# KrishTanna28/Real-Time-Video-Deepfake-Detection

Hardware: AMD Instinct MI355X
Metric: face-crops/sec (224x224 crops through EfficientNet-B0 classify) (higher is better)
Workload: dtype f32; 1 GPU; configs[1]: batch=256 random 224x224 crops, EfficientNet-B0 fp32 inference; batch_per_gpu=256, parallelism=frame-shard x1, no data-path collective, forwards_in_flight=2

## Files before the change

### real-time-video-deepfake-detection_amd/csrc/b0_kernels.h

```cpp
#pragma once
#include <hip/hip_runtime.h>

#include <string>

namespace dfd {

typedef __bf16 bf16_t;

enum Act { ACT_NONE = 0, ACT_SWISH = 1, ACT_RELU = 2, ACT_PRELU = 3 };

template <typename XT>
void launch_stem(const float* x_nchw, const float* w , const float* b,
                 XT* y, int n, hipStream_t s);

template <typename XT>
void launch_stem_dw(const float* x_nchw, const unsigned short* ws3, int plane, int Kp, const float* bs, const float* Wd,
                    const float* bd, XT* Y, float* P, XT* stem_out, int n, int* tiles, hipStream_t s);

void launch_pointwise(const float* X, const float* W, const float* bias, const float* gate,
                      const float* R, float* Y, int M, int K, int N, int HW, int act,
                      hipStream_t s);

struct ConvGeom {
    int H = 0, W = 0, Ho = 0, Wo = 0, Cin = 0, ksize = 1, stride = 1, pad = 0, dil = 1;
};

bool launch_conv_gemm(const float* X, const float* W, const float* bias, const float* R, float* Y,
                      int n_img, const ConvGeom& g, int Cout, int act, bool res_first, hipStream_t s);

size_t split_weights_count(int N, int K);
void launch_split_weights(const float* W, unsigned short* out, int N, int K, hipStream_t s, bool transposed = false);
bool split_gemm_supports(int K, int N);
bool split_gemm_thin_supports(int K, int N, int HW);
struct S6Table;
S6Table* s6_table_create();
void s6_table_destroy(S6Table* t);
void s6_table_set_force(S6Table* t, int idx);
void s6_table_set_tuning(S6Table* t, bool on);
int s6_table_measured(const S6Table* t);
int s6_max_candidates();
long long s6_chunk_rows(long long M, long long row_bytes, long long HW);
std::string s6_table_export(const S6Table* t);
int s6_table_import(S6Table* t, const char* text, size_t len);
template <typename XT>
bool launch_pointwise_split(S6Table* tab, const XT* X, const unsigned short* W3, const float* bias, const float* gate,
                            const XT* R, XT* Y, int M, int K, int N, int HW, int act, int planes, hipStream_t s);
template <typename XT>
bool launch_conv_gemm_split(S6Table* tab, const XT* X, const unsigned short* W3, const float* bias, const XT* R,
                            XT* Y, int n_img, const ConvGeom& g, int Cout, int act, bool res_first, int planes, hipStream_t s);

template <typename XT>
bool launch_depthwise(const XT* X, const float* W , const float* bias, XT* Y,
                      float* P, int n, int H, int C, int k, int stride, int pad_lo,
                      int* tiles, hipStream_t s);
int depthwise_tiles(int H, int C, int k, int stride);
template <typename XT>
bool launch_mbconv_front(const XT* Xin, int Cin, const unsigned short* We3, int plane, int Kp, const float* Wef, const float* be,
                         const float* Wd, const float* bd, XT* Y, float* P, int n, int H, int C, int k, int stride,
                         int pad_lo, int* tiles, hipStream_t s, bool late = false);
int mbconv_tiles(int H, int C, int k, int stride, int Cin, bool late = false);

void launch_se(const float* P, int tiles, float inv_hw, const float* w1, const float* b1,
               const float* w2t, const float* b2, float* gate, int n, int C, int c_se,
               hipStream_t s);

template <typename XT>
void launch_avgpool(const XT* X, float* Y, int n, int hw, int C, hipStream_t s);
void launch_bf16_to_f32(const bf16_t* x, float* y, size_t n, hipStream_t s);

}
```

### real-time-video-deepfake-detection_amd/csrc/b0_plan.hip

```cpp
#include <algorithm>

#include "b0_kernels.h"
#include "dfd_common.h"

namespace dfd {

thread_local std::string g_create_error;

int fail(dfd_handle* h, int code, const char* fmt, ...) {
    char buf[512];
    va_list ap;
    va_start(ap, fmt);
    vsnprintf(buf, sizeof buf, fmt, ap);
    va_end(ap);
    if (h) h->err = buf;
    else g_create_error = buf;
    return code;
}

namespace {

struct Stage { int rep, k, s, e, ci, co; };
const Stage kStages[] = {{1, 3, 1, 1, 32, 16}, {2, 3, 2, 6, 16, 24}, {2, 5, 2, 6, 24, 40},
                         {3, 3, 2, 6, 40, 80}, {3, 5, 1, 6, 80, 112}, {4, 5, 2, 6, 112, 192},
// ... 187 lines not shown
    }
    if ((rc = tap_out(h, tap, "stem", io0, (size_t)n * 112 * 112 * 32))) return rc;
    XT* cur = io0;
    XT* nxt = io1;
    int bi = 0;
    for (const B0Block& b : P.blocks) {
        const int m_in = n * b.h_in * b.h_in, m_out = n * b.h_out * b.h_out;
        const std::string q = "b" + std::to_string(bi);
        const XT* dw_in = cur;
        int tiles = 0;
        bool fused = false;
        const unsigned short* we3 = nullptr;
        const bool late_here = h->fuse_late && !((h->fuse_late_skip >> bi) & 1u);
        if (b.expand != 1 && h->fuse_expand && mbconv_tiles(b.h_in, b.c_exp, b.kernel, b.stride, b.c_in, late_here) > 0 &&
            !(we3 = split_weights(h, b.exp_w, b.c_exp, b.c_in))) return DFD_ERR_HIP;
        if (we3 && launch_mbconv_front<XT>(cur, b.c_in, we3, (int)split_weights_count(b.c_exp, b.c_in), (b.c_in + 63) / 64 * 64,
                                           b.exp_w, b.exp_b, b.dw_w, b.dw_b, dwbuf, h->pool, n, b.h_in, b.c_exp,
                                           b.kernel, b.stride, b.pad_lo, &tiles, s, late_here)) {
            fused = true;
            mk.mark(layer_name(bi, "dw"));
            if (tap && tap->name && q + ".exp" == tap->name)
                return fail(h, DFD_ERR_STATE, "tap '%s': the expanded tensor is not materialised when expand is fused "
                                              "(dfd_set_option(h, \"fuse_expand\", 0))", tap->name);
        }
        if (!fused && b.expand != 1) {
            if ((rc = pointwise_t<XT>(h, cur, b.exp_w, b.exp_b, nullptr, nullptr, expbuf, m_in, b.c_in, b.c_exp,
                                      b.h_in * b.h_in, ACT_SWISH))) return rc;
            mk.mark(layer_name(bi, "exp"));
            if ((rc = tap_out(h, tap, q + ".exp", expbuf, (size_t)m_in * b.c_exp))) return rc;
            dw_in = expbuf;
        }
        if (bi == 0 && stem_fused) {
            tiles = stem_tiles;
        } else if (!fused) {
            if (!launch_depthwise<XT>(dw_in, b.dw_w, b.dw_b, dwbuf, h->pool, n, b.h_in, b.c_exp, b.kernel,
                                      b.stride, b.pad_lo, &tiles, s))
                return fail(h, DFD_ERR_STATE, "no depthwise kernel for block %d", bi);
            mk.mark(layer_name(bi, "dw"));
        }
        if ((rc = tap_out(h, tap, q + ".dw", dwbuf, (size_t)m_out * b.c_exp))) return rc;
        launch_se(h->pool, tiles, 1.0f / (float)(b.h_out * b.h_out), b.se_w1, b.se_b1, b.se_w2, b.se_b2,
                  h->gate, n, b.c_exp, b.c_se, s);
        mk.mark(layer_name(bi, "se"));
        if ((rc = tap_out(h, tap, q + ".gate", h->gate, (size_t)n * b.c_exp))) return rc;
        if ((rc = pointwise_t<XT>(h, dwbuf, b.proj_w, b.proj_b, h->gate, b.skip ? cur : (const XT*)nullptr, nxt, m_out,
                                  b.c_exp, b.c_out, b.h_out * b.h_out, ACT_NONE))) return rc;
        mk.mark(layer_name(bi, "proj"));
        if ((rc = tap_out(h, tap, q + ".out", nxt, (size_t)m_out * b.c_out))) return rc;
        XT* t = cur; cur = nxt; nxt = t;
        ++bi;
    }
    const B0Block& last = P.blocks.back();
    const int hw = last.h_out * last.h_out;
    if ((rc = pointwise_t<XT>(h, cur, P.head_w, P.head_b, nullptr, nullptr, headbuf, n * hw, last.c_out, 1280, hw,
                              ACT_SWISH))) return rc;
    mk.mark("head");
    if ((rc = tap_out(h, tap, "head", headbuf, (size_t)n * hw * 1280))) return rc;
    launch_avgpool<XT>(headbuf, h->feat, n, hw, 1280, s);
    mk.mark("avgpool");
    if ((rc = tap_out(h, tap, "feat", h->feat, (size_t)n * 1280))) return rc;
    if (!logits_dev) return DFD_OK;
    if ((rc = pointwise(h, h->feat, P.fc1_w, P.fc1_b, nullptr, nullptr, h->fc1, n, 1280, 512, 1, ACT_RELU))) return rc;
    if ((rc = pointwise(h, h->fc1, P.fc2_w, P.fc2_b, nullptr, nullptr, h->fc2, n, 512, 256, 1, ACT_RELU))) return rc;
    launch_pointwise(h->fc2, P.fc3_w, P.fc3_b, nullptr, nullptr, logits_dev, n, 256, 1, 1, ACT_NONE, s);
    mk.mark("mlp");
    if ((rc = tap_out(h, tap, "logit", logits_dev, (size_t)n))) return rc;
    DFD_HIP_TRY(h, hipGetLastError());
    return DFD_OK;
}

float* b0_last_block_out(const dfd_handle* h) { return h->b0.blocks.size() % 2 == 0 ? h->io0 : h->io1; }

int b0_head_preact(dfd_handle* h, int n, void* z_out) {
    const B0Plan& P = h->b0;
    const B0Block& last = P.blocks.back();
    const int hw = last.h_out * last.h_out;
    if (h->act_bf16)
        return pointwise_t<bf16_t>(h, reinterpret_cast<const bf16_t*>(b0_last_block_out(h)), P.head_w, P.head_b, nullptr, nullptr,
                                   static_cast<bf16_t*>(z_out), n * hw, last.c_out, 1280, hw, ACT_NONE);
    return pointwise_t<float>(h, b0_last_block_out(h), P.head_w, P.head_b, nullptr, nullptr, static_cast<float*>(z_out),
                              n * hw, last.c_out, 1280, hw, ACT_NONE);
}

int b0_forward(dfd_handle* h, const float* x, int n, float* logits_dev, B0Tap* tap, B0Prof* prof) {
    if (n > 0) h->classifier_crops += (unsigned long long)n;
    return h->act_bf16 ? b0_forward_t<bf16_t>(h, x, n, logits_dev, tap, prof)
                       : b0_forward_t<float>(h, x, n, logits_dev, tap, prof);
}

}
```

### real-time-video-deepfake-detection_amd/csrc/dfd_api.hip

```cpp
#include "b0_kernels.h"
#include "dfd_common.h"

using namespace dfd;

namespace {

int dev_alloc(dfd_handle* h, size_t bytes, float** out) {
    void* p = nullptr;
    DFD_HIP_TRY(h, hipMalloc(&p, bytes ? bytes : 4));
    h->owned.push_back(p);
    *out = static_cast<float*>(p);
    return DFD_OK;
}

__global__ __launch_bounds__(256) void fill_pattern_kernel(float* __restrict__ x, size_t n) {
    const size_t i = (size_t)blockIdx.x * 256 + threadIdx.x;
    if (i >= n) return;
    uint32_t v = (uint32_t)i * 2654435761u;
    v ^= v >> 15; v *= 2246822519u; v ^= v >> 13;
    x[i] = ((float)(v >> 8) * (1.0f / 16777216.0f) - 0.5f) * 4.0f;
}

int create_impl(dfd_handle* h, int device, const void* blob, size_t blob_len, int max_batch) {
    int ndev = 0;
// ... 83 lines not shown
    }
    h->jpeg_stream = nullptr;
    if (h->aux_stream) {
        hipStreamSynchronize(h->aux_stream);
        hipStreamDestroy(h->aux_stream);
        hipEventDestroy(h->aux_go);
        hipEventDestroy(h->aux_done);
    }
    if (h->jpeg_host) hipHostFree(h->jpeg_host);
    if (h->mailbox) hipHostFree(h->mailbox);
    for (char* p : h->mailbox_old) hipHostFree(p);
    for (char* p : h->mailbox_old_prev) hipHostFree(p);
    if (h->ev0) hipEventDestroy(h->ev0);
    if (h->order_ev) hipEventDestroy(h->order_ev);
    if (h->ev1) hipEventDestroy(h->ev1);
    if (h->stream) hipStreamDestroy(h->stream);
    delete h;
}

}

extern "C" {

int dfd_abi_version(void) { return DFD_ABI_VERSION; }

int dfd_create(int device, const void* blob, size_t blob_len, int max_batch, dfd_handle** out) {
    if (!out) return fail(nullptr, DFD_ERR_ARG, "dfd_create: out is null");
    *out = nullptr;
    if (!blob || max_batch <= 0 || max_batch > 4096)
        return fail(nullptr, DFD_ERR_ARG, "dfd_create: blob is null or max_batch outside 1..4096");
    dfd_handle* h = new (std::nothrow) dfd_handle();
    if (!h) return fail(nullptr, DFD_ERR_ARG, "dfd_create: out of host memory");
    const int rc = create_impl(h, device, blob, blob_len, max_batch);
    if (rc != DFD_OK) {
        g_create_error = h->err;
        destroy_impl(h);
        return rc;
    }
    *out = h;
    return DFD_OK;
}

void dfd_destroy(dfd_handle* h) { destroy_impl(h); }

const char* dfd_last_error(const dfd_handle* h) { return h ? h->err.c_str() : g_create_error.c_str(); }

int dfd_max_batch(const dfd_handle* h) { return h ? h->max_batch : DFD_ERR_ARG; }

int dfd_set_option(dfd_handle* h, const char* name, int value) {
    if (!h || !name) return DFD_ERR_ARG;
    if (strcmp(name, "fuse_expand") == 0) { h->fuse_expand = value != 0; return DFD_OK; }
    if (strcmp(name, "fuse_late") == 0) { h->fuse_late = value != 0; return DFD_OK; }
    if (strcmp(name, "fuse_late_skip") == 0) { h->fuse_late_skip = (unsigned)value; return DFD_OK; }
    if (strcmp(name, "fuse_stem") == 0) { h->fuse_stem = value != 0; return DFD_OK; }
    if (strcmp(name, "split_gemm") == 0) { h->split_gemm = value != 0; return DFD_OK; }
    if (strcmp(name, "mtcnn") == 0) { h->use_mtcnn = value != 0; return DFD_OK; }
    if (strcmp(name, "overlap_forensics") == 0) { h->overlap_forensics = value != 0; return DFD_OK; }
    if (strcmp(name, "bf16_activations") == 0) { h->act_bf16 = value != 0; return DFD_OK; }
    if (strcmp(name, "bf16_weight_planes") == 0) {
        if (value != 1 && value != 3) return fail(h, DFD_ERR_ARG, "bf16_weight_planes must be 1 or 3");
        h->bf16_planes = value;
        return DFD_OK;
    }
    if (strcmp(name, "gemm_tile") == 0) { s6_table_set_force(h->gemm, value); return DFD_OK; }
    if (strcmp(name, "jpeg_device_entropy") == 0) { h->jpeg_device_entropy = value < 0 ? 0 : value; return DFD_OK; }
    if (strcmp(name, "jpeg_rounds") == 0) { h->jpeg_rounds = value; return DFD_OK; }
    if (strcmp(name, "jpeg_chunk_bytes") == 0) {
        if (value < 256 || value > (1 << 20) || (value & (value - 1))) return fail(h, DFD_ERR_ARG, "jpeg_chunk_bytes: a power of two in 256 .. 2^20");
        h->jpeg_chunk_bytes = value;
        return DFD_OK;
    }
    if (strcmp(name, "stream_priority") == 0) {
        if (value < -1 || value > 1) return fail(h, DFD_ERR_ARG, "stream_priority must be -1, 0 or 1");
        DFD_HIP_TRY(h, hipSetDevice(h->device));
        DFD_HIP_TRY(h, stream_sync(h));
        if (h->aux_stream) DFD_HIP_TRY(h, hipStreamSynchronize(h->aux_stream));
        if (h->copy_stream) DFD_HIP_TRY(h, hipStreamSynchronize(h->copy_stream));
        int least = 0, greatest = 0;
        DFD_HIP_TRY(h, hipDeviceGetStreamPriorityRange(&least, &greatest));
        const int prio = value > 0 ? greatest : (value < 0 ? least : (least + greatest) / 2);
        hipStream_t fresh = nullptr;
        DFD_HIP_TRY(h, hipStreamCreateWithPriority(&fresh, hipStreamNonBlocking, prio));
        hipStreamDestroy(h->stream);
        h->stream = fresh;
        return DFD_OK;
    }
    if (strcmp(name, "profile_stride") == 0) { h->prof_stride = value > 0 ? value : 1; return DFD_OK; }
    return fail(h, DFD_ERR_ARG, "unknown option '%s'", name);
}

int dfd_warmup(dfd_handle* h, int n_crops, int n_frames) {
    if (!h) return DFD_ERR_ARG;
    if (n_crops < 0 || n_crops > h->max_batch || n_frames < 0)
        return fail(h, DFD_ERR_ARG, "warmup: n_crops outside 0..%d or n_frames negative", h->max_batch);
    DFD_HIP_TRY(h, hipSetDevice(h->device));
    s6_table_set_tuning(h->gemm, true);
    int rc = DFD_OK;
    if (n_crops > 0) {
        const size_t cnt = (size_t)n_crops * 3 * 224 * 224;
        hipLaunchKernelGGL(fill_pattern_kernel, dim3((unsigned)((cnt + 255) / 256)), dim3(256), 0, h->stream, h->in_nchw, cnt);
        rc = b0_forward(h, h->in_nchw, n_crops, h->logits, nullptr, nullptr);
    }
    if (rc == DFD_OK && n_frames > 0) rc = ssd_warmup(h, n_frames);
    s6_table_set_tuning(h->gemm, false);
    if (rc) return rc;
    DFD_HIP_TRY(h, stream_sync(h));
// ... 192 lines not shown
```

### real-time-video-deepfake-detection_amd/csrc/dfd_common.h

```cpp
#pragma once
#include <hip/hip_runtime.h>

#include <cstdarg>
#include <cstdint>
#include <cstdio>
#include <cstring>
#include <map>
#include <string>
#include <vector>

#include "../../include/dfd_hip.h"
#include "blob_reader.h"
#include "imgproc_kernels.h"

namespace dfd {

struct ForensicState;
void forensic_destroy(dfd_handle* h);
struct FreqState;
void freq_destroy(dfd_handle* h);
struct SsdState;
int ssd_init(dfd_handle* h);
void ssd_destroy(dfd_handle* h);
int ssd_warmup(dfd_handle* h, int n_frames);
// ... 33 lines not shown
    float* out = nullptr;
    size_t capacity = 0, count = 0;
    bool found = false;
};
struct B0Prof {
    std::vector<hipEvent_t> events;
    std::vector<const char*> names;
    bool enabled = false;
};

}

struct dfd_handle {
    int device = 0;
    int max_batch = 0;
    hipStream_t stream = nullptr;
    hipEvent_t ev0 = nullptr, ev1 = nullptr;
    hipEvent_t order_ev = nullptr;
    char* mailbox = nullptr;
    size_t mailbox_cap = 0, mailbox_head = 0, mailbox_lap_end = 0;
    size_t mailbox_live = 0, mailbox_live_prev = 0;
    std::vector<char*> mailbox_old, mailbox_old_prev;
    hipStream_t aux_stream = nullptr;
    hipEvent_t aux_go = nullptr, aux_done = nullptr;
    bool overlap_forensics = true;
    hipStream_t copy_stream = nullptr;
    hipEvent_t copy_done[2] = {nullptr, nullptr}, slot_free[2] = {nullptr, nullptr};
    dfd::DevBuf stage[2];
    std::map<std::string, dfd::Tensor> tensors;
    std::vector<void*> owned;
    dfd::B0Plan b0;
    float *in_nchw = nullptr, *io0 = nullptr, *io1 = nullptr, *expbuf = nullptr, *dwbuf = nullptr;
    float *pool = nullptr, *gate = nullptr, *headbuf = nullptr, *feat = nullptr, *fc1 = nullptr,
          *fc2 = nullptr, *logits = nullptr;
    dfd::ColorTables color{};
    bool has_color = false;
    dfd::DevBuf frame_buf, lab_buf, crop_buf, lut_buf, desc_buf, u8_out, face_batch;
    dfd::DevBuf det_desc;
    int last_detections = 0;
    std::vector<char> crop_valid;
    int n_compact = 0;
    unsigned long long classifier_crops = 0;
    dfd::ForensicState* forensic = nullptr;
    dfd::FreqState* freq = nullptr;
    dfd::SsdState* ssd = nullptr;
    dfd::MtcnnState* mtcnn = nullptr;
    dfd::HaarState* haar = nullptr;
    dfd::CommState* comm = nullptr;
    bool use_mtcnn = true;
    bool fuse_stem = true;
    bool fuse_expand = true;
    bool fuse_late = true;
    unsigned fuse_late_skip = (1u << 8) | (1u << 9);
    bool split_gemm = true;
    bool act_bf16 = false;
    int bf16_planes = 3;
    dfd::DevBuf jpeg_work;
    dfd::DevBuf jpeg_raw[2];
    dfd::DevBuf jpeg_work2[2];
    hipStream_t jpeg_stream = nullptr;
    hipEvent_t jpeg_done[2] = {nullptr, nullptr}, frames_free[2] = {nullptr, nullptr};
    void* jpeg_host = nullptr;
    size_t jpeg_host_cap = 0;
    int jpeg_device_entropy = 2;
    int jpeg_rounds = 16;
    int jpeg_chunk_bytes = 512;
    unsigned long long jpeg_frames_device = 0, jpeg_frames_host = 0;
    dfd::DevBuf tap_buf;
    std::map<const float*, unsigned short*> wsplit;
    dfd::S6Table* gemm = nullptr;
    dfd::B0Prof prof;
    int prof_steps = 0;
    int prof_seen = 0, prof_stride = 1;
    std::string err;
};

namespace dfd {

extern thread_local std::string g_create_error;

int fail(dfd_handle* h, int code, const char* fmt, ...);

#define DFD_HIP_TRY(h, expr)                                                                    \
    do {                                                                                        \
        hipError_t _e = (expr);                                                                 \
        if (_e != hipSuccess)                                                                   \
            return dfd::fail((h), DFD_ERR_HIP, "%s failed: %s (%s:%d)", #expr, hipGetErrorString(_e), \
                             __FILE__, __LINE__);                                               \
    } while (0)

int ensure(dfd_handle* h, DevBuf* b, size_t bytes);
hipError_t stream_sync(dfd_handle* h);
int mailbox_h2d(dfd_handle* h, void* dst_dev, const void* src, size_t bytes);
const void* mailbox_d2h(dfd_handle* h, const void* src_dev, size_t bytes);
void copy_kernel_async(void* dst, const void* src, size_t bytes, hipStream_t s);
int color_tables_init(dfd_handle* h);

int forensics_run(dfd_handle* h, int stream_id, const uint8_t* frame_dev, int hh, int ww, int stride, int full,
                  double* scores_out, double* prob_out, double* stats_out);
int detect_run(dfd_handle* h, const uint8_t* frame_dev, int hh, int ww, int stride, float conf_thr, int32_t* xywh_out,
               float* conf_out, int max_out, int* n_out);
int haar_run(dfd_handle* h, const uint8_t* frame_dev, int hh, int ww, int stride, float scale_factor, int min_neighbors,
             int min_size, int32_t* xywh_out, int max_out, int* n_out, int* n_candidates, int* n_total = nullptr);
int preprocess_run(dfd_handle* h, const uint8_t* frame_dev, int hh, int ww, int stride, const int32_t* xywh, int n,
                   int apply_clahe, const size_t* frame_offs = nullptr, bool compact = false);
int classify_boxes(dfd_handle* h, const uint8_t* frame_dev, int hh, int ww, int stride, const int32_t* xywh, int m,
// ... 38 lines not shown
```

### real-time-video-deepfake-detection_amd/csrc/gemm_split.hip

```cpp
#include "gemm_split_impl.h"

#include <algorithm>
#include <cmath>
#include <cstdio>
#include <cstdlib>
#include <map>
#include <new>
#include <string>
#include <tuple>
#include <vector>

namespace dfd {

DFD_S6_INSTANTIATE(float, 3)

__global__ __launch_bounds__(256) void split_weights_kernel(const float* __restrict__ W, __bf16* __restrict__ out,
                                                            int N, int K, int Np, int Kp, int transposed) {
    const size_t i = (size_t)blockIdx.x * 256 + threadIdx.x, plane = (size_t)Np * Kp;
    if (i >= plane) return;
    const int n = (int)(i / Kp), k = (int)(i - (size_t)n * Kp);
    const float a = n < N && k < K ? (transposed ? W[(size_t)k * N + n] : W[(size_t)n * K + k]) : 0.f;
    const __bf16 h0 = (__bf16)a;
    const float r1 = a - (float)h0;
    const __bf16 h1 = (__bf16)r1;
// ... 35 lines not shown
            const double blocks = (double)t.mblocks * t.nblocks;
            const double useful = (double)tiles / ((double)t.nblocks * nt);
            const double rounds = std::max(1.0, std::ceil(blocks / 512.0));
            const double cost = rounds * (mt * nt + 1.5) / useful;
            if (cost < best_cost - 1e-9) { best_cost = cost; best = t; }
        }
    return best;
}

static std::vector<S6Tile> s6_candidates(int M, int K, int N, bool thin = false, bool wide = false) {
    const int tiles = (N + 15) / 16;
    std::vector<S6Tile> raw, out;
    for (int ks = 1; ks <= (K > 32 ? 2 : 1); ++ks)
        for (int mt = 1; mt <= 2; ++mt)
            for (int nt = 1; nt <= 8 && nt <= tiles; ++nt) raw.push_back(make_tile6(M, N, mt, nt, ks));
    for (int ks = 1; ks <= (K > 32 ? 2 : 1); ++ks)
        for (int nt = 2; nt <= 8 && nt <= tiles; ++nt) raw.push_back(make_tile(M, N, 0, 8, 1, 1, nt, ks));
#define DFD_S7_CAND(WMV, WNV, MTV, NTV) raw.push_back(make_tile(M, N, 1, WMV, WNV, MTV, NTV));
    DFD_S7_CONFIGS(DFD_S7_CAND)
#undef DFD_S7_CAND
    for (const S6Tile& t : raw) {
        const int bn_tiles = t.kind == 0 ? t.nt : t.wn * t.nt;
        if ((double)tiles / ((double)t.nblocks * bn_tiles) < 0.7) continue;
        if ((long long)t.mblocks * t.nblocks > (1 << 20)) continue;
        out.push_back(t);
    }
    if (out.empty()) out.push_back(make_tile6(M, N, 1, 1));
    if (wide)
    {
        for (int nt : {6, 4}) out.push_back(make_tile(M, N, 3, 4, 1, 2, nt, 1));
        out.push_back(make_tile(M, N, 3, 4, 1, 2, 4, 2));
    }
    if (thin)
        for (int bpc : {2, 3, 4, 6, 8, 12, 16, 24}) out.push_back(make_tile(M, N, 2, s8_waves(K), 1, 1, tiles, bpc));
    return out;
}

struct S6Key {
    int M, K, N, mode;
    bool operator<(const S6Key& o) const {
        return std::tie(M, K, N, mode) < std::tie(o.M, o.K, o.N, o.mode);
    }
};
struct S6Table {
    std::map<S6Key, S6Tile> tiles;
    int force = -1;
    bool tuning = false;
};

S6Table* s6_table_create() { return new (std::nothrow) S6Table(); }
void s6_table_destroy(S6Table* t) { delete t; }
void s6_table_set_force(S6Table* t, int idx) { if (t) t->force = idx; }
void s6_table_set_tuning(S6Table* t, bool on) { if (t) t->tuning = on; }
int s6_table_measured(const S6Table* t) {
    int n = 0;
    if (t) for (const auto& kv : t->tiles) n += kv.second.measured ? 1 : 0;
    return n;
}
std::string s6_table_export(const S6Table* t) {
    std::string out;
    if (!t) return out;
    char line[128];
    for (const auto& kv : t->tiles) {
        if (!kv.second.measured) continue;
        snprintf(line, sizeof line, "%d %d %d %d %d %d %d %d %d %d\n", kv.first.M, kv.first.K, kv.first.N, kv.first.mode,
                 kv.second.kind, kv.second.wm, kv.second.wn, kv.second.mt, kv.second.nt, kv.second.ks);
        out += line;
    }
    return out;
}
int s6_table_import(S6Table* t, const char* text, size_t len) {
    if (!t || !text) return -1;
    int n = 0;
    const std::string all(text, len);
    size_t pos = 0;
    while (pos < all.size()) {
        size_t e = all.find('\n', pos);
        if (e == std::string::npos) e = all.size();
        int v[10];
        if (sscanf(all.substr(pos, e - pos).c_str(), "%d %d %d %d %d %d %d %d %d %d", &v[0], &v[1], &v[2], &v[3], &v[4], &v[5],
                   &v[6], &v[7], &v[8], &v[9]) == 10) {
            bool known = false;
            for (const S6Tile& c : s6_candidates(v[0], v[1], v[2], (v[3] & 128) != 0, (v[3] & 64) != 0))
                known |= c.kind == v[4] && c.wm == v[5] && c.wn == v[6] && c.mt == v[7] && c.nt == v[8] && c.ks == v[9];
            if (known) {
                S6Tile tile = make_tile(v[0], v[2], v[4], v[5], v[6], v[7], v[8], v[9]);
                tile.measured = true;
                t->tiles[S6Key{v[0], v[1], v[2], v[3]}] = tile;
                ++n;
            }
        }
        pos = e + 1;
    }
    return n;
}

int s6_max_candidates() { return (int)s6_candidates(1 << 20, 1152, 1280).size(); }

long long s6_chunk_rows(long long M, long long row_bytes, long long HW) {
    const long long lim = (1ll << 31) - 1;
    if (HW <= 0) HW = 1;
    if (M * row_bytes <= lim) return M;
    long long imgs = lim / (row_bytes * HW);
    if (imgs < 1) return -1;
    return imgs * HW;
}
// ... 77 lines not shown
    if constexpr (sizeof(XT) == 2) {
        if (planes == 1) {
            s6_run_one<XT, 1>(tab, conv, gated, X, W3, bias, gate, R, Y, M, K, N, HW, act, g, res_first, s);
            return;
        }
    }
    s6_run_one<XT, 3>(tab, conv, gated, X, W3, bias, gate, R, Y, M, K, N, HW, act, g, res_first, s);
}

bool split_gemm_supports(int K, int N) { return K % 8 == 0 && K >= 16 && split_weights_count(N, K) * 6 < (1ull << 31); }

template <typename XT>
bool launch_pointwise_split(S6Table* tab, const XT* X, const unsigned short* W3, const float* bias, const float* gate,
                            const XT* R, XT* Y, int M, int K, int N, int HW, int act, int planes, hipStream_t s) {
    const ConvGeom none{};
    if (HW <= 0) HW = 1;
    const long long chunk = s6_chunk_rows(M, (long long)K * (long long)sizeof(XT), gate ? HW : 1);
    if (chunk <= 0) return false;
    for (long long m0 = 0; m0 < M; m0 += chunk) {
        const int mc = (int)std::min<long long>(chunk, M - m0);
        s6_run_np<XT>(planes, tab, false, gate != nullptr, X + (size_t)m0 * K, W3, bias,
                      gate ? gate + (size_t)(m0 / HW) * K : nullptr, R ? R + (size_t)m0 * N : nullptr, Y + (size_t)m0 * N,
                      mc, K, N, HW, act, none, 0, s);
    }
    return true;
}
template bool launch_pointwise_split<float>(S6Table*, const float*, const unsigned short*, const float*, const float*,
                                            const float*, float*, int, int, int, int, int, int, hipStream_t);
template bool launch_pointwise_split<bf16_t>(S6Table*, const bf16_t*, const unsigned short*, const float*, const float*,
                                             const bf16_t*, bf16_t*, int, int, int, int, int, int, hipStream_t);

template <typename XT>
bool launch_conv_gemm_split(S6Table* tab, const XT* X, const unsigned short* W3, const float* bias, const XT* R,
                            XT* Y, int n_img, const ConvGeom& g, int Cout, int act, bool res_first, int planes, hipStream_t s) {
    if (g.Cin % S6_BK != 0) return false;
    const int K = g.ksize * g.ksize * g.Cin;
    if (!split_gemm_supports(K, Cout)) return false;
    const long long in_img = (long long)g.H * g.W * g.Cin * (long long)sizeof(XT), out_rows = (long long)g.Ho * g.Wo;
    const long long imgs = s6_chunk_rows(n_img, in_img, 1);
    if (imgs <= 0) return false;
    for (long long i0 = 0; i0 < n_img; i0 += imgs) {
        const int ni = (int)std::min<long long>(imgs, n_img - i0);
        s6_run_np<XT>(planes, tab, true, false, X + (size_t)i0 * g.H * g.W * g.Cin, W3, bias, nullptr,
                      R ? R + (size_t)i0 * out_rows * Cout : nullptr, Y + (size_t)i0 * out_rows * Cout,
                      (int)(ni * out_rows), K, Cout, 1, act, g, res_first ? 1 : 0, s);
    }
    return true;
}
template bool launch_conv_gemm_split<float>(S6Table*, const float*, const unsigned short*, const float*, const float*, float*,
                                            int, const ConvGeom&, int, int, bool, int, hipStream_t);
template bool launch_conv_gemm_split<bf16_t>(S6Table*, const bf16_t*, const unsigned short*, const float*, const bf16_t*,
                                             bf16_t*, int, const ConvGeom&, int, int, bool, int, hipStream_t);

#ifdef S6_TRACE
extern "C" int dfd_debug_s6_trace(long long* out, int n) {
    return (int)hipMemcpyFromSymbol(out, HIP_SYMBOL(g_s6_trace), (size_t)n * sizeof(long long), 0, hipMemcpyDeviceToHost);
}
#endif

}
```

### real-time-video-deepfake-detection_amd/csrc/gemm_split_bf16.hip

```cpp
#include "gemm_split_impl.h"

namespace dfd {

DFD_S6_INSTANTIATE(bf16_t, 3)
DFD_S6_INSTANTIATE(bf16_t, 1)

}
```

### real-time-video-deepfake-detection_amd/csrc/gemm_split_impl.h

```cpp
#pragma once
#include "b0_kernels.h"
#include "kernel_util.h"

#include <type_traits>

namespace dfd {


#ifdef S6_TRACE
#ifndef S6_TRACE_K
#define S6_TRACE_K 1152
#endif
#ifndef S6_TRACE_N
#define S6_TRACE_N 192
#endif
__device__ long long g_s6_trace[1024];
#define S6_TP(id)                                                                                          \
    do {                                                                                                   \
        if (K == S6_TRACE_K && N == S6_TRACE_N && blockIdx.x == 8 && threadIdx.x == 0 && tp < 1000) {      \
            g_s6_trace[tp++] = (long long)(id);                                                            \
            g_s6_trace[tp++] = (long long)__builtin_amdgcn_s_memtime();                                    \
        }                                                                                                  \
    } while (0)
#else
// ... 933 lines not shown
        auto body = [&](auto cur_c, int nb, bool have_prev) {
            constexpr int cur = decltype(cur_c)::value;
#pragma unroll
            for (int mt = 0; mt < MT; ++mt)
#pragma unroll
                for (int nt = 0; nt < NT; ++nt) accs[cur][mt][nt] = (v4f){0.f, 0.f, 0.f, 0.f};
#pragma unroll
            for (int ks = 0; ks < NKC; ++ks, ++stage) {
                const int nks = ks + 1 < NKC ? ks + 1 : 0, nnb = ks + 1 < NKC ? nb : (nb + 1 < nblocks ? nb + 1 : nb);
                load_w(nnb, nks);
                const unsigned char* wb = ws[stage & 1];
                bf8 wf[2][3];
                read_w(wb, 0, wf[0]);
#pragma unroll
                for (int nt = 0; nt < NT; ++nt) {
                    if (nt + 1 < NT) read_w(wb, nt + 1, wf[(nt + 1) & 1]);
                    s6_products<MT, 3, 3, NT>(accs[cur], xs[ks], wf[nt & 1], nt);
#pragma unroll
                    for (int i = 0; i < TPS; ++i) {
                        if (((i + 1) * NT + TPS - 1) / TPS - 1 == nt) {
                            const int e = ks * TPS + i;
                            if (e < TILES && have_prev) {
                                const int pn = e / MT, pm = e - pn * MT;
                                finish_tile(accs[cur ^ 1][pm][pn], bvp[pn], pm, (nb - 1) * BN + pn * 16 + 4 * q);
                            }
                        }
                    }
                }
                store_w((stage + 1) & 1);
                __syncthreads();
            }
            load_bias(nb, bvp);
        };
        int nb = 0;
        for (; nb + 2 <= nblocks; nb += 2) {
            body(std::integral_constant<int, 0>{}, nb, nb > 0);
            body(std::integral_constant<int, 1>{}, nb + 1, true);
        }
        if (nb < nblocks) {
            body(std::integral_constant<int, 0>{}, nb, nb > 0);
            ++nb;
        }
        const int last = (nblocks - 1) & 1;
#pragma unroll
        for (int nt = 0; nt < NT; ++nt)
#pragma unroll
            for (int mt = 0; mt < MT; ++mt) {
                if (last == 0) finish_tile(accs[0][mt][nt], bvp[nt], mt, (nblocks - 1) * BN + nt * 16 + 4 * q);
                else finish_tile(accs[1][mt][nt], bvp[nt], mt, (nblocks - 1) * BN + nt * 16 + 4 * q);
            }
    }
}

#define DFD_S9_NK_CASES(OP) OP(3) OP(4)
inline bool s9_supports(int K, int N) {
    const int nk = (K + S6_BK - 1) / S6_BK;
    return K % 8 == 0 && (nk == 3 || nk == 4) && N >= 192 && N % 4 == 0;
}

#define DFD_S8_NK_CASES(OP) OP(1, 4) OP(3, 4) OP(5, 4) OP(8, 8)
inline int s8_waves(int K) { return (K + S6_BK - 1) / S6_BK == 8 ? 8 : 4; }
inline bool s8_supports(int K, int N) {
    const int nk = (K + S6_BK - 1) / S6_BK;
    return N % 4 == 0 && N <= 48 && K % 8 == 0 && (nk == 1 || nk == 3 || nk == 5 || nk == 8);
}

struct S6Tile { int kind, wm, wn, mt, nt, ks, mblocks, nblocks; bool measured; };
inline S6Tile make_tile(int M, int N, int kind, int wm, int wn, int mt, int nt, int ks = 1) {
    const int bm = wm * mt * 16, bn = wn * nt * 16;
    return S6Tile{kind, wm, wn, mt, nt, ks, (M + bm - 1) / bm, (N + bn - 1) / bn, false};
}
inline S6Tile make_tile6(int M, int N, int mt, int nt, int ks = 1) { return make_tile(M, N, 0, 4, 1, mt, nt, ks); }

#define DFD_S6_NT_CASES(OP) OP(1) OP(2) OP(3) OP(4) OP(5) OP(6) OP(7) OP(8)
#define DFD_S7_CONFIGS(OP)                                                                       \
    OP(1, 4, 2, 1) OP(1, 4, 2, 2) OP(1, 4, 2, 3) OP(1, 4, 4, 1) OP(1, 4, 4, 2) OP(1, 4, 4, 3)     \
    OP(2, 2, 1, 2) OP(2, 2, 1, 3) OP(2, 2, 1, 4) OP(2, 2, 1, 6) OP(2, 2, 2, 2) OP(2, 2, 2, 3)     \
    OP(2, 2, 2, 4) OP(2, 2, 2, 6) OP(2, 2, 4, 2) OP(2, 2, 4, 3)

template <bool CONV, bool GATE, typename XT, int NP>
void s6_dispatch(const S6Tile& t, const XT* X, const unsigned short* W3, const float* bias,
                 const float* gate, const XT* R, XT* Y, int M, int K, int N, int HW, int act,
                 const ConvGeom& g, int res_first, hipStream_t s) {
    const int grid = ((t.mblocks + 7) / 8) * 8 * t.nblocks;
    const int Kp = (K + S6_KPAD - 1) / S6_KPAD * S6_KPAD, plane = s6_np(N) * Kp;
    const unsigned xbytes = CONV ? (unsigned)((size_t)(M / (g.Ho * g.Wo)) * g.H * g.W * g.Cin * sizeof(XT))
                                 : (unsigned)((size_t)M * K * sizeof(XT));
    const unsigned gbytes = GATE ? (unsigned)((size_t)((M + HW - 1) / HW) * K * 4) : 0u;
    if (t.kind == 3) {
        if constexpr (!CONV && !GATE && sizeof(XT) == 4 && NP == 3) {
            const int nk = (K + S6_BK - 1) / S6_BK, mb = (M + 127) / 128;
#define DFD_S9_CASE(NKV)                                                                                                     \
    if (nk == NKV) {                                                                                                         \
        if (t.nt == 6 && t.ks == 1) hipLaunchKernelGGL((pw9_kernel<6, NKV, false, XT, NP>), dim3(mb), dim3(256), 0, s, X, W3, plane, Kp, \
                                                       bias, Y, M, K, N, act, xbytes);                                       \
        else if (t.ks == 1) hipLaunchKernelGGL((pw9_kernel<4, NKV, false, XT, NP>), dim3(mb), dim3(256), 0, s, X, W3, plane, Kp, bias, \
                                               Y, M, K, N, act, xbytes);                                                     \
        else hipLaunchKernelGGL((pw9_kernel<4, NKV, true, XT, NP>), dim3(mb), dim3(256), 0, s, X, W3, plane, Kp, bias, Y, M, K, \
                                N, act, xbytes);                                                                             \
    }
            DFD_S9_NK_CASES(DFD_S9_CASE)
#undef DFD_S9_CASE
        }
        return;
    }
    if (t.kind == 2) {
// ... 69 lines not shown
```

Before: 95160 crops/s.

## Fuse head 1x1 conv, swish, and global average pool into one kernel

Adds a head_pool kernel that computes the 320->1280 head pointwise GEMM with bias and swish, then reduces over the 7x7 spatial positions in shared memory and writes pooled features directly. This skips writing and re-reading the full n*49*1280 head activation buffer and removes the separate avgpool launch. It is on by default behind a new fuse_head_pool option, falling back to the old path when a tap of the head output is requested or during tile tuning. The fused kernel uses a fixed tile shape (2 images per block, 10 N-tiles), which may give lower GEMM efficiency than the tuned split GEMM.

```diff
diff --git a/profiles/head_pool_probe.py b/profiles/head_pool_probe.py
--- /dev/null
+++ b/profiles/head_pool_probe.py
@@ -0,0 +1,54 @@
+import os
+import sys
+import time
+
+import numpy as np
+
+ROOT = os.path.dirname(os.path.dirname(os.path.abspath(__file__)))
+sys.path.insert(0, ROOT)
+import rtdfd_amd
+
+W = rtdfd_amd.weights
+PAIRS, STEPS = int(os.environ.get("HP_PAIRS", "5")), int(os.environ.get("HP_STEPS", "50"))
+SETTINGS = (0, 1)
+h = rtdfd_amd._lib.Handle(W.pack_b0(W.seeded_state_dict(0)), device=0, max_batch=256)
+h.set_option("bf16_activations", int(os.environ.get("B0_BF16", "0")))
+x = np.random.RandomState(1).randn(256, 3, 224, 224).astype(np.float32)
+xd = h.alloc(x.nbytes).upload(x)
+yd = h.alloc(1024)
+h.warmup(256, 0)
+logits = {}
+for s in SETTINGS:
+    h.set_option("fuse_head_pool", s)
+    for _ in range(5):
+        h.classify_device(xd.ptr, 256, yd.ptr)
+    h.sync()
+    logits[s] = yd.download((256, 1))
+print("logits bit-equal across settings:", all(np.array_equal(logits[s], logits[0]) for s in SETTINGS))
+
+ms = {s: [] for s in SETTINGS}
+for r in range(PAIRS):
+    for s in SETTINGS:
+        h.set_option("fuse_head_pool", s)
+        h.classify_device(xd.ptr, 256, yd.ptr)
+        h.sync()
+        t0 = time.perf_counter()
+        for _ in range(STEPS):
+            h.classify_device(xd.ptr, 256, yd.ptr)
+        h.sync()
+        ms[s].append((time.perf_counter() - t0) / STEPS * 1e3)
+for s in SETTINGS:
+    v = ms[s]
+    print(f"fuse_head_pool={s}: ms per forward {' '.join(f'{t:.4f}' for t in v)}  median {np.median(v):.4f}")
+
+for s in SETTINGS:
+    h.set_option("fuse_head_pool", s)
+    h.profile_begin()
+    for _ in range(20):
+        h.classify_device(xd.ptr, 256, yd.ptr)
+    seen, layers = h.profile_end()
+    kinds = {k: sum(t for n, t in layers if n == k) / seen * 1e3 for k in ("head", "avgpool", "mlp")}
+    total = sum(t for _, t in layers) / seen
+    print(f"fuse_head_pool={s}: per-launch events over {seen} forwards: head {kinds['head']:.1f} us, avgpool {kinds['avgpool']:.1f} us, "
+          f"mlp {kinds['mlp']:.1f} us, all launches {total:.3f} ms")
+h.close()
diff --git a/real-time-video-deepfake-detection_amd/csrc/b0_kernels.h b/real-time-video-deepfake-detection_amd/csrc/b0_kernels.h
--- a/real-time-video-deepfake-detection_amd/csrc/b0_kernels.h
+++ b/real-time-video-deepfake-detection_amd/csrc/b0_kernels.h
@@ -37,6 +37,7 @@
 void s6_table_destroy(S6Table* t);
 void s6_table_set_force(S6Table* t, int idx);
 void s6_table_set_tuning(S6Table* t, bool on);
+bool s6_table_tuning(const S6Table* t);
 int s6_table_measured(const S6Table* t);
 int s6_max_candidates();
 long long s6_chunk_rows(long long M, long long row_bytes, long long HW);
@@ -48,6 +49,11 @@
 template <typename XT>
 bool launch_conv_gemm_split(S6Table* tab, const XT* X, const unsigned short* W3, const float* bias, const XT* R,
                             XT* Y, int n_img, const ConvGeom& g, int Cout, int act, bool res_first, int planes, hipStream_t s);
+
+bool head_pool_supports(int n_img, int HW, int K, int N, size_t elem_bytes);
+template <typename XT>
+void launch_head_pool(const XT* X, const unsigned short* W3, const float* bias, float* feat, int n_img, int HW, int K, int N,
+                      int planes, hipStream_t s);
 
 template <typename XT>
 bool launch_depthwise(const XT* X, const float* W , const float* bias, XT* Y,
diff --git a/real-time-video-deepfake-detection_amd/csrc/b0_plan.hip b/real-time-video-deepfake-detection_amd/csrc/b0_plan.hip
--- a/real-time-video-deepfake-detection_amd/csrc/b0_plan.hip
+++ b/real-time-video-deepfake-detection_amd/csrc/b0_plan.hip
@@ -263,12 +263,23 @@
     }
     const B0Block& last = P.blocks.back();
     const int hw = last.h_out * last.h_out;
-    if ((rc = pointwise_t<XT>(h, cur, P.head_w, P.head_b, nullptr, nullptr, headbuf, n * hw, last.c_out, 1280, hw,
-                              ACT_SWISH))) return rc;
-    mk.mark("head");
-    if ((rc = tap_out(h, tap, "head", headbuf, (size_t)n * hw * 1280))) return rc;
-    launch_avgpool<XT>(headbuf, h->feat, n, hw, 1280, s);
-    mk.mark("avgpool");
+    const bool want_head = tap && tap->name && std::string(tap->name) == "head";
+    const bool pooled = h->fuse_head_pool && !want_head && (sizeof(XT) == 2 || h->split_gemm) &&
+                        head_pool_supports(n, hw, last.c_out, 1280, sizeof(XT));
+    if (!pooled || s6_table_tuning(h->gemm)) {
+        if ((rc = pointwise_t<XT>(h, cur, P.head_w, P.head_b, nullptr, nullptr, headbuf, n * hw, last.c_out, 1280, hw,
+                                  ACT_SWISH))) return rc;
+        mk.mark("head");
+        if ((rc = tap_out(h, tap, "head", headbuf, (size_t)n * hw * 1280))) return rc;
+        launch_avgpool<XT>(headbuf, h->feat, n, hw, 1280, s);
+        mk.mark("avgpool");
+    }
+    if (pooled) {
+        const unsigned short* wh3 = split_weights(h, P.head_w, 1280, last.c_out);
+        if (!wh3) return DFD_ERR_HIP;
+        launch_head_pool<XT>(cur, wh3, P.head_b, h->feat, n, hw, last.c_out, 1280, sizeof(XT) == 2 ? h->bf16_planes : 3, s);
+        mk.mark("head");
+    }
     if ((rc = tap_out(h, tap, "feat", h->feat, (size_t)n * 1280))) return rc;
     if (!logits_dev) return DFD_OK;
     if ((rc = pointwise(h, h->feat, P.fc1_w, P.fc1_b, nullptr, nullptr, h->fc1, n, 1280, 512, 1, ACT_RELU))) return rc;
diff --git a/real-time-video-deepfake-detection_amd/csrc/dfd_api.hip b/real-time-video-deepfake-detection_amd/csrc/dfd_api.hip
--- a/real-time-video-deepfake-detection_amd/csrc/dfd_api.hip
+++ b/real-time-video-deepfake-detection_amd/csrc/dfd_api.hip
@@ -159,6 +159,7 @@
     if (strcmp(name, "fuse_expand") == 0) { h->fuse_expand = value != 0; return DFD_OK; }
     if (strcmp(name, "fuse_late") == 0) { h->fuse_late = value != 0; return DFD_OK; }
     if (strcmp(name, "fuse_late_skip") == 0) { h->fuse_late_skip = (unsigned)value; return DFD_OK; }
+    if (strcmp(name, "fuse_head_pool") == 0) { h->fuse_head_pool = value != 0; return DFD_OK; }
     if (strcmp(name, "fuse_stem") == 0) { h->fuse_stem = value != 0; return DFD_OK; }
     if (strcmp(name, "split_gemm") == 0) { h->split_gemm = value != 0; return DFD_OK; }
     if (strcmp(name, "mtcnn") == 0) { h->use_mtcnn = value != 0; return DFD_OK; }
diff --git a/real-time-video-deepfake-detection_amd/csrc/dfd_common.h b/real-time-video-deepfake-detection_amd/csrc/dfd_common.h
--- a/real-time-video-deepfake-detection_amd/csrc/dfd_common.h
+++ b/real-time-video-deepfake-detection_amd/csrc/dfd_common.h
@@ -109,6 +109,7 @@
     bool fuse_expand = true;
     bool fuse_late = true;
     unsigned fuse_late_skip = (1u << 8) | (1u << 9);
+    bool fuse_head_pool = true;
     bool split_gemm = true;
     bool act_bf16 = false;
     int bf16_planes = 3;
diff --git a/real-time-video-deepfake-detection_amd/csrc/gemm_split.hip b/real-time-video-deepfake-detection_amd/csrc/gemm_split.hip
--- a/real-time-video-deepfake-detection_amd/csrc/gemm_split.hip
+++ b/real-time-video-deepfake-detection_amd/csrc/gemm_split.hip
@@ -111,6 +111,7 @@
 void s6_table_destroy(S6Table* t) { delete t; }
 void s6_table_set_force(S6Table* t, int idx) { if (t) t->force = idx; }
 void s6_table_set_tuning(S6Table* t, bool on) { if (t) t->tuning = on; }
+bool s6_table_tuning(const S6Table* t) { return t && t->tuning; }
 int s6_table_measured(const S6Table* t) {
     int n = 0;
     if (t) for (const auto& kv : t->tiles) n += kv.second.measured ? 1 : 0;
@@ -294,6 +295,15 @@
 template bool launch_conv_gemm_split<bf16_t>(S6Table*, const bf16_t*, const unsigned short*, const float*, const bf16_t*,
                                              bf16_t*, int, const ConvGeom&, int, int, bool, int, hipStream_t);
 
+bool head_pool_supports(int n_img, int HW, int K, int N, size_t elem_bytes) {
+    return head_pool_shape_ok(n_img, HW, K, N, HP_NT * 16, elem_bytes) && split_gemm_supports(K, N);
+}
+template <>
+void launch_head_pool<float>(const float* X, const unsigned short* W3, const float* bias, float* feat, int n_img, int HW, int K,
+                             int N, int planes, hipStream_t s) {
+    head_pool_dispatch<float, 3>(X, W3, bias, feat, n_img, HW, K, N, s);
+}
+
 #ifdef S6_TRACE
 extern "C" int dfd_debug_s6_trace(long long* out, int n) {
     return (int)hipMemcpyFromSymbol(out, HIP_SYMBOL(g_s6_trace), (size_t)n * sizeof(long long), 0, hipMemcpyDeviceToHost);
diff --git a/real-time-video-deepfake-detection_amd/csrc/gemm_split_bf16.hip b/real-time-video-deepfake-detection_amd/csrc/gemm_split_bf16.hip
--- a/real-time-video-deepfake-detection_amd/csrc/gemm_split_bf16.hip
+++ b/real-time-video-deepfake-detection_amd/csrc/gemm_split_bf16.hip
@@ -5,4 +5,11 @@
 DFD_S6_INSTANTIATE(bf16_t, 3)
 DFD_S6_INSTANTIATE(bf16_t, 1)
 
+template <>
+void launch_head_pool<bf16_t>(const bf16_t* X, const unsigned short* W3, const float* bias, float* feat, int n_img, int HW, int K,
+                              int N, int planes, hipStream_t s) {
+    if (planes == 1) head_pool_dispatch<bf16_t, 1>(X, W3, bias, feat, n_img, HW, K, N, s);
+    else head_pool_dispatch<bf16_t, 3>(X, W3, bias, feat, n_img, HW, K, N, s);
 }
+
+}
diff --git a/real-time-video-deepfake-detection_amd/csrc/gemm_split_impl.h b/real-time-video-deepfake-detection_amd/csrc/gemm_split_impl.h
--- a/real-time-video-deepfake-detection_amd/csrc/gemm_split_impl.h
+++ b/real-time-video-deepfake-detection_amd/csrc/gemm_split_impl.h
@@ -1009,6 +1009,153 @@
     }
 }
 
+constexpr int HP_NK = 10, HP_HW = 49;
+template <int NT, typename XT, int NP>
+__global__ __launch_bounds__(256, 2) void head_pool_kernel(const XT* __restrict__ X, const unsigned short* __restrict__ W3,
+                                                                           int plane, int Kp, const float* __restrict__ bias,
+                                                                           float* __restrict__ F, int n_img, int HW, int N,
+                                                                           unsigned xbytes) {
+    constexpr int BK = S6_BK, NK = HP_NK, K = NK * BK, MT = 2, BN = NT * 16, NW = 4, NTHR = NW * 64, IPW = NW / 2;
+    constexpr int ESZ = (int)sizeof(XT), XL = ESZ == 4 ? 2 : 1, NXS = ESZ == 4 ? 3 : 1;
+    static_assert(NP == 3 || (NP == 1 && ESZ == 2), "weight planes: 3 (fp32-exact), or 1 with bf16 activations");
+    constexpr int CHUNKS = BN * 4 * NP, WLOADS = (CHUNKS + NTHR - 1) / NTHR;
+    constexpr int PS = BN + 4;
+    constexpr int WS_STAGE = BN * S6_ROWB, PS_BYTES = IPW * HP_HW * PS * 4;
+    __shared__ __attribute__((aligned(16))) unsigned char smem[2 * WS_STAGE > PS_BYTES ? 2 * WS_STAGE : PS_BYTES];
+
+    const int tid = threadIdx.x, wave = tid >> 6, lane = tid & 63, j = lane & 15, q = lane >> 4;
+    const int nparts = N / BN, cpart = blockIdx.x % nparts, img0 = (blockIdx.x / nparts) * IPW;
+    const int n0 = cpart * BN, il = wave >> 1, half = wave & 1;
+
+    const __amdgpu_buffer_rsrc_t rw = __builtin_amdgcn_make_buffer_rsrc(const_cast<unsigned short*>(W3), 0, 6 * plane, 0x00020000);
+    const __amdgpu_buffer_rsrc_t rx = __builtin_amdgcn_make_buffer_rsrc(const_cast<XT*>(X), 0, xbytes, 0x00020000);
+    int wvo[WLOADS], wlds[WLOADS];
+#pragma unroll
+    for (int t = 0; t < WLOADS; ++t) {
+        const int e = tid + t * NTHR < CHUNKS ? tid + t * NTHR : CHUNKS - 1;
+        const int row = e / (4 * NP), rem = e - row * (4 * NP), pl = rem >> 2, c = rem & 3;
+        wvo[t] = 2 * (pl * plane + (n0 + row) * Kp + 8 * c);
+        wlds[t] = row * S6_ROWB + s6_chunk_pos(row, pl * 4 + c) * 16;
+    }
+    int xvo[MT];
+#pragma unroll
+    for (int mt = 0; mt < MT; ++mt) {
+        const int r = half * 32 + mt * 16 + j, img = img0 + il < n_img ? img0 + il : n_img - 1;
+        xvo[mt] = ESZ * ((img * HW + (r < HW ? r : HW - 1)) * K + 8 * q);
+    }
+    u4 wr[WLOADS];
+    v4f xr[3][MT][XL];
+    auto load_w = [&](int ks) {
+#pragma unroll
+        for (int t = 0; t < WLOADS; ++t) wr[t] = __builtin_amdgcn_raw_buffer_load_b128(rw, wvo[t], 2 * ks * BK, 0);
+    };
+    auto store_w = [&](int buf) {
+#pragma unroll
+        for (int t = 0; t < WLOADS; ++t) *reinterpret_cast<u4*>(smem + buf * WS_STAGE + wlds[t]) = wr[t];
+    };
+    auto load_x = [&](int ks, v4f (&x)[MT][XL]) {
+#pragma unroll
+        for (int mt = 0; mt < MT; ++mt) {
+            x[mt][0] = __builtin_bit_cast(v4f, __builtin_amdgcn_raw_buffer_load_b128(rx, xvo[mt], ESZ * BK * ks, 0));
+            if constexpr (XL == 2) x[mt][1] = __builtin_bit_cast(v4f, __builtin_amdgcn_raw_buffer_load_b128(rx, xvo[mt] + 16, ESZ * BK * ks, 0));
+        }
+    };
+
+    v4f acc[MT][NT];
+#pragma unroll
+    for (int mt = 0; mt < MT; ++mt)
+#pragma unroll
+        for (int nt = 0; nt < NT; ++nt) acc[mt][nt] = (v4f){0.f, 0.f, 0.f, 0.f};
+
+    const int rd0 = s6_chunk_pos(j, q) * 16, rd1 = s6_chunk_pos(j, 4 + q) * 16, rd2 = s6_chunk_pos(j, 8 + q) * 16;
+    auto compute = [&](const v4f (&x)[MT][XL], const unsigned char* wb) {
+        bf8 xs[MT][NXS];
+#pragma unroll
+        for (int mt = 0; mt < MT; ++mt) {
+            if constexpr (ESZ == 4) split8(x[mt][0], x[mt][XL - 1], xs[mt][0], xs[mt][NXS > 1 ? 1 : 0], xs[mt][NXS > 2 ? 2 : 0]);
+            else xs[mt][0] = __builtin_bit_cast(bf8, x[mt][0]);
+        }
+        bf8 wf[2][NP];
+        auto read_w = [&](int nt, bf8 (&f)[NP]) {
+            const unsigned char* wp = wb + (nt * 16 + j) * S6_ROWB;
+            f[0] = *reinterpret_cast<const bf8*>(wp + rd0);
+            if constexpr (NP == 3) {
+                f[1] = *reinterpret_cast<const bf8*>(wp + rd1);
+                f[2] = *reinterpret_cast<const bf8*>(wp + rd2);
+            }
+        };
+        read_w(0, wf[0]);
+#pragma unroll
+        for (int nt = 0; nt < NT; ++nt) {
+            if (nt + 1 < NT) read_w(nt + 1, wf[(nt + 1) & 1]);
+            __builtin_amdgcn_sched_barrier(0);
+            s6_products<MT, NXS, NP, NT>(acc, xs, wf[nt & 1], nt);
+            __builtin_amdgcn_sched_barrier(0);
+        }
+    };
+
+    load_w(0);
+    load_x(0, xr[0]);
+    load_x(1, xr[1]);
+    store_w(0);
+    __syncthreads();
+#pragma unroll
+    for (int ks = 0; ks < NK; ++ks) {
+        if (ks + 1 < NK) load_w(ks + 1);
+        if (ks + 2 < NK) load_x(ks + 2, xr[(ks + 2) % 3]);
+        __builtin_amdgcn_sched_barrier(0);
+        compute(xr[ks % 3], smem + (ks & 1) * WS_STAGE);
+        __builtin_amdgcn_sched_barrier(0);
+        if (ks + 1 < NK) store_w((ks + 1) & 1);
+        __syncthreads();
+    }
+
+    float* ps = reinterpret_cast<float*>(smem);
+#pragma unroll
+    for (int nt = 0; nt < NT; ++nt) {
+        const v4f bv = ldg4(bias + n0 + nt * 16 + 4 * q);
+#pragma unroll
+        for (int mt = 0; mt < MT; ++mt) {
+            v4f v = swish4(acc[mt][nt] + bv);
+            if constexpr (ESZ == 2) v = __builtin_convertvector(__builtin_convertvector(v, bf4v), v4f);
+            const int r = half * 32 + mt * 16 + j;
+            if (r < HW) stg4(ps + (il * HW + r) * PS + nt * 16 + 4 * q, v);
+        }
+    }
+    __syncthreads();
+    constexpr int Q = BN / 4, ITEMS = IPW * Q;
+    const int part = lane >> 3;
+    const float inv = 1.0f / (float)HW;
+    for (int it = wave; it * 8 < ITEMS; it += NW) {
+        const int item = it * 8 + (lane & 7);
+        const bool live = item < ITEMS;
+        const int ic = live ? item : 0, li = ic / Q, c = (ic - li * Q) * 4;
+        v4f s = (v4f){0.f, 0.f, 0.f, 0.f};
+        for (int i = part; i < HW; i += 8) s += ldg4(ps + (li * HW + i) * PS + c);
+#pragma unroll
+        for (int off = 8; off < 64; off <<= 1) {
+            s.x += __shfl_xor(s.x, off);
+            s.y += __shfl_xor(s.y, off);
+            s.z += __shfl_xor(s.z, off);
+            s.w += __shfl_xor(s.w, off);
+        }
+        if (live && part == 0 && img0 + li < n_img) stg4(F + (size_t)(img0 + li) * N + n0 + c, s * inv);
+    }
+}
+
+inline bool head_pool_shape_ok(int n_img, int HW, int K, int N, int bn, size_t esz) {
+    return n_img > 0 && HW > 0 && HW <= HP_HW && K == HP_NK * S6_BK && N % bn == 0 && (size_t)n_img * HW * K * esz < (1ull << 31);
+}
+constexpr int HP_NT = 10;
+template <typename XT, int NP>
+void head_pool_dispatch(const XT* X, const unsigned short* W3, const float* bias, float* F, int n_img, int HW, int K, int N,
+                        hipStream_t s) {
+    const int Kp = (K + S6_KPAD - 1) / S6_KPAD * S6_KPAD, plane = s6_np(N) * Kp;
+    const unsigned xbytes = (unsigned)((size_t)n_img * HW * K * sizeof(XT));
+    hipLaunchKernelGGL((head_pool_kernel<HP_NT, XT, NP>), dim3((n_img + 1) / 2 * (N / (HP_NT * 16))), dim3(256), 0, s, X, W3, plane, Kp,
+                       bias, F, n_img, HW, N, xbytes);
+}
+
 #define DFD_S9_NK_CASES(OP) OP(3) OP(4)
 inline bool s9_supports(int K, int N) {
     const int nk = (K + S6_BK - 1) / S6_BK;
```

Result: no change. 94620 crops/s (-0.6%).
